# facebookresearch/localrf

Measured on AMD Instinct MI355X. Metric: rays/sec (4096-ray batch, 512 samples, 300^3 grid), higher is better.
Workload: dtype f32 (colour network: split-bf16 3-term products on v_mfma_f32_32x32x16_bf16, fp32 accumulate, <= 3e-5 vs the exact-fp32 engine; gathers and compositing fp32); 1 GPU; configs[1]: single 300^3 TensorVMSplit, 4096 rays x 512 samples per GPU, full density+appearance+MLP render, eval forward; rays_per_gpu=4096, samples_per_ray=512, grid=300, parallelism=ray-shard x1, mlp_engine=bf16x3

## Files before the change

include/lrf_debug.h:

```cpp
#ifndef LRF_DEBUG_H_
#define LRF_DEBUG_H_

#include <stdint.h>

#ifdef __cplusplus
extern "C" {
#endif

void    lrf_debug_set_dump(float* buf);
void    lrf_debug_set_lds_lines(int on);
void    lrf_debug_set_pipe_chunk(int rays);
void    lrf_debug_set_scene_fuse(int on);
void    lrf_debug_set_bwd_overlap(int on);
void    lrf_debug_set_train_fwd_engine(int bits);
void    lrf_debug_set_scatter_wgs(int n);
int64_t lrf_debug_saved_row_offset(int buffer, uint64_t row, int col);

#ifdef __cplusplus
}
#endif
#endif
```

localrf_amd/_native.py:

```python
import ctypes as C
import os

_HERE = os.path.dirname(os.path.abspath(__file__))
LIB_PATH = os.environ.get("LRF_LIB", os.path.join(_HERE, "csrc", "liblrf_hip.so"))

LRF_FLAG_WHITE_BG = 1
LRF_FLAG_RELU_DENS = 2
LRF_FLAG_MLP_VALU = 4
LRF_FLAG_MLP_F32 = 8
LRF_FLAG_ROWS_SAVED = 16
LRF_FLAG_SORT_RAYS = 32
LRF_FLAG_PE_OFF = 64
LRF_FLAG_PLANE_EVENTS = 128
LRF_FLAG_DETERMINISTIC = 256
LRF_FLAG_ALL = 511

_f = C.c_void_p


class LrfParams(C.Structure):
    _fields_ = [("density_plane", _f * 3), ("density_line", _f * 3),
                ("app_plane", _f * 3), ("app_line", _f * 3),
                ("basis", _f), ("w1", _f), ("b1", _f), ("w2", _f), ("b2", _f), ("w3", _f), ("b3", _f),
                ("grid", C.c_int32 * 3), ("fea_pe", C.c_int32), ("view_pe", C.c_int32), ("feature_c", C.c_int32)]
# ... 35 lines not shown

class LrfFlowLoss(C.Structure):
    _fields_ = [("cam2world", _f), ("frame", C.c_void_p), ("fwd_off", C.c_void_p), ("dirs", _f), ("depth", _f), ("ij", C.c_void_p),
                ("fwd_flow", _f), ("fwd_mask", _f), ("bwd_flow", _f), ("bwd_mask", _f), ("focal", _f), ("center", _f),
                ("F", C.c_int32), ("V", C.c_int32), ("n", C.c_int32), ("quantile", C.c_float)]


LRF_LOSS_MAX_PER_VIEW = 4096
LRF_LOSS_TERMS_MAX = 8


class LrfBatchGather(C.Structure):
    _fields_ = [("images", _f), ("fwd_flow", _f), ("bwd_flow", _f), ("invdepths", _f), ("view_ids", C.c_void_p), ("pix", C.c_void_p),
                ("V", C.c_int32), ("n", C.c_int32), ("HW", C.c_int32), ("n_images", C.c_int32)]


class LrfLossTerms(C.Structure):
    _fields_ = [("x", _f * LRF_LOSS_TERMS_MAX), ("n", C.c_int32 * LRF_LOSS_TERMS_MAX), ("a", C.c_float * LRF_LOSS_TERMS_MAX),
                ("b", C.c_float * LRF_LOSS_TERMS_MAX), ("count", C.c_int32), ("s", _f)]


class LrfImageMetrics(C.Structure):
    _fields_ = [("img0", _f), ("img1", _f), ("B", C.c_int32), ("H", C.c_int32), ("W", C.c_int32), ("filter_size", C.c_int32),
                ("max_val", C.c_double), ("filter_sigma", C.c_double), ("k1", C.c_double), ("k2", C.c_double)]


LRF_FRAMES_ERR_NOT_RESIDENT = 1


class LrfFrameWindow(C.Structure):
    _fields_ = [("rgb", _f), ("loss_weight", _f), ("invdepth", _f), ("fwd_flow", _f), ("fwd_mask", _f), ("bwd_flow", _f),
                ("bwd_mask", _f), ("slot_of", C.c_void_p), ("status", C.c_void_p),
                ("capacity", C.c_int32), ("n_px", C.c_int32), ("num_images", C.c_int32)]


LRF_SELECT_QUANTILE = 0
LRF_SELECT_MEDIAN = 1
LRF_SELECT_MAX_ROWS = 256
LRF_EVAL_MAX_VIEWS = 64


class LrfFlowComparison(C.Structure):
    _fields_ = [("cam2world", _f), ("depth", _f), ("dirs", _f), ("ij", C.c_void_p), ("fwd_flow", _f), ("fwd_mask", _f),
                ("bwd_flow", _f), ("bwd_mask", _f), ("focal", _f), ("center", _f),
                ("F", C.c_int32), ("V", C.c_int32), ("H", C.c_int32), ("W", C.c_int32), ("idx", C.c_int32 * LRF_EVAL_MAX_VIEWS)]


SYMBOLS = {
    "lrf_abi_version": (C.c_int, []),
    "lrf_last_error": (C.c_char_p, []),
    "lrf_error_slot": (C.c_void_p, []),
    "lrf_debug_set_dump": (None, [C.c_void_p]),
    "lrf_debug_set_lds_lines": (None, [C.c_int]),
    "lrf_debug_set_pipe_chunk": (None, [C.c_int]),
    "lrf_debug_set_scene_fuse": (None, [C.c_int]),
    "lrf_debug_saved_row_offset": (C.c_int64, [C.c_int, C.c_uint64, C.c_int]),
    "lrf_debug_set_bwd_overlap": (None, [C.c_int]),
    "lrf_debug_set_train_fwd_engine": (None, [C.c_int]),
    "lrf_debug_set_scatter_wgs": (None, [C.c_int]),
    "lrf_workspace_layout_bwd": (None, [C.c_int32, C.c_int32, C.POINTER(C.c_int32), C.POINTER(C.c_uint64)]),
    "lrf_cache_bytes": (C.c_size_t, [C.POINTER(C.c_int32)]),
    "lrf_pack_field": (C.c_int, [C.POINTER(LrfParams), C.c_void_p, C.c_void_p]),
    "lrf_workspace_bytes": (C.c_size_t, [C.c_int32, C.c_int32]),
    "lrf_render_fwd": (C.c_int, [C.POINTER(LrfField), _f, _f, C.c_int32, C.c_int32, C.c_uint32, C.c_float,
                                 _f, _f, _f, _f, C.c_void_p, C.c_void_p]),
    "lrf_render_fwd_profile": (C.c_int, [C.POINTER(LrfField), _f, _f, C.c_int32, C.c_int32, C.c_uint32,
                                         C.c_float, _f, _f, C.c_void_p, C.c_void_p,
                                         C.POINTER(C.c_float), C.POINTER(C.c_int32)]),
    "lrf_render_fwd_train": (C.c_int, [C.POINTER(LrfField), _f, _f, C.c_int32, C.c_int32, C.c_uint32, _f, _f,
                                       C.c_void_p, C.c_void_p]),
    "lrf_workspace_bytes_bwd": (C.c_size_t, [C.c_int32, C.c_int32, C.POINTER(C.c_int32)]),
    "lrf_workspace_bytes_bwd_cfg": (C.c_size_t, [C.c_int32, C.c_int32, C.POINTER(C.c_int32), C.c_int32, C.c_int32, C.c_int32, C.c_uint32]),
    "lrf_render_bwd": (C.c_int, [C.POINTER(LrfField), C.POINTER(LrfParams), _f, _f, C.c_int32, C.c_int32,
                                 C.c_uint32, _f, _f, C.POINTER(LrfGrads), _f, C.c_void_p, C.c_void_p]),
    "lrf_render_bwd_wait": (C.c_int, [C.c_int32, C.c_void_p]),
    "lrf_density_feature": (C.c_int, [C.POINTER(LrfField), _f, C.c_int32, _f, C.c_void_p]),
    "lrf_app_feature": (C.c_int, [C.POINTER(LrfField), _f, C.c_int32, _f, C.c_void_p]),
    "lrf_sample_ray_aabb": (C.c_int, [_f, C.POINTER(C.c_float), C.c_float, C.c_float, C.c_float, _f,
                                      C.c_int32, C.c_int32, _f, _f, C.c_void_p, C.c_void_p]),
    "lrf_sample_ray_contracted": (C.c_int, [_f, _f, _f, C.c_int32, C.c_int32, _f, C.c_void_p]),
    "lrf_z_schedule": (C.c_int, [C.c_int32, _f, _f, _f, C.c_void_p]),
    "lrf_adam_step": (C.c_int, [C.POINTER(LrfAdamTensor), C.c_int32, C.c_float, C.c_float, C.c_float, C.c_void_p]),
    "lrf_adam_step_pack": (C.c_int, [C.POINTER(LrfAdamTensor), C.c_int32, _f, C.c_float, C.c_float, C.c_float, C.POINTER(LrfParams), C.c_void_p, C.c_void_p]),
    "lrf_photo_loss_fwd": (C.c_int, [_f, _f, _f, _f, C.c_int32, _f, _f, C.c_void_p]),
    "lrf_photo_loss_bwd": (C.c_int, [_f, _f, _f, _f, _f, C.c_int32, _f, C.c_void_p]),
    "lrf_batch_gather": (C.c_int, [C.POINTER(LrfBatchGather), _f, _f, _f, _f, _f, _f, C.c_void_p]),
    "lrf_loss_combine_fwd": (C.c_int, [C.POINTER(LrfLossTerms), _f, _f, C.c_void_p]),
    "lrf_loss_combine_bwd": (C.c_int, [_f, _f, C.c_int32, _f, C.c_void_p]),
    "lrf_rows_gather": (C.c_int, [_f, C.c_void_p, C.c_int32, C.c_int32, C.c_int32, _f, C.c_void_p]),
    "lrf_rows_gather_bwd": (C.c_int, [_f, C.c_void_p, C.c_int32, C.c_int32, C.c_int32, _f, C.c_void_p]),
    "lrf_adam_step_dev": (C.c_int, [C.POINTER(LrfAdamTensor), C.c_int32, _f, C.c_float, C.c_float, C.c_float, C.c_void_p]),
    "lrf_density_l1_workspace": (C.c_size_t, [C.POINTER(C.c_int32), C.POINTER(C.c_int32)]),
    "lrf_density_l1_fwd": (C.c_int, [C.POINTER(_f), C.POINTER(_f), C.POINTER(C.c_int32), C.POINTER(C.c_int32),
                                     C.c_float, C.c_int32, C.c_void_p, _f, C.c_void_p]),
    "lrf_density_l1_bwd": (C.c_int, [C.POINTER(_f), C.POINTER(_f), C.POINTER(C.c_int32), C.POINTER(C.c_int32),
                                     C.c_void_p, _f, C.POINTER(_f), C.POINTER(_f), C.c_void_p]),
    "lrf_density_l1_bwd_acc": (C.c_int, [C.POINTER(_f), C.POINTER(_f), C.POINTER(C.c_int32), C.POINTER(C.c_int32),
                                     C.c_void_p, _f, C.POINTER(_f), C.POINTER(_f), C.c_void_p]),
    "lrf_pose_assemble": (C.c_int, [C.POINTER(_f), C.POINTER(_f), C.c_int32, C.c_int32, _f, C.c_void_p]),
    "lrf_pose_assemble_bwd": (C.c_int, [C.POINTER(_f), C.c_int32, C.c_int32, _f, _f, _f, C.c_void_p]),
    "lrf_dense_alpha": (C.c_int, [C.POINTER(LrfField), _f, _f, _f, C.c_int32, C.c_int32, C.c_int32, C.c_float,
                                  C.c_uint32, _f, C.c_void_p]),
    "lrf_alpha_pool_threshold": (C.c_int, [_f, C.c_int32, C.c_int32, C.c_int32, C.c_float, _f, C.c_void_p]),
    "lrf_tv_workspace": (C.c_size_t, [C.POINTER(LrfTvSeg), C.c_int32]),
    "lrf_tv_loss_fwd": (C.c_int, [C.POINTER(LrfTvSeg), C.c_int32, C.c_float, C.c_void_p, _f, C.c_void_p]),
    "lrf_tv_loss_bwd": (C.c_int, [C.POINTER(LrfTvSeg), C.c_int32, C.c_float, _f, C.c_void_p]),
# ... 72 lines not shown
```

localrf_amd/csrc/lrf_common.h:

```cpp
#pragma once
#include "lrf_tu.h"
#include <hip/hip_runtime.h>
#include <stdint.h>
#include "../../include/lrf.h"

namespace lrf {

constexpr int MAT0[3] = {0, 0, 1};
constexpr int MAT1[3] = {1, 2, 2};
constexpr int VEC[3]  = {2, 1, 0};

constexpr int LRF_CAS = 32;
__host__ __device__ constexpr int app_pc(int c) { return 8 * (c / 6) + c % 6; }

constexpr int IMG_BAS  = 0;
constexpr int IMG_W1   = IMG_BAS + 2 * 3 * 64 * 8;
constexpr int IMG_W2   = IMG_W1 + 8 * 2 * 64 * 4;
constexpr int IMG_W3H  = IMG_W2 + 8 * 8 * 64 * 4;
constexpr int IMG_B1   = IMG_W3H + 4 * 32 * 4;
constexpr int IMG_B2   = IMG_B1 + 128;
constexpr int IMG_W3V  = IMG_B2 + 128;
constexpr int IMG_FLOATS = IMG_W3V + 16;

constexpr int IMGB_BAS = 0;
// ... 57 lines not shown
  return (row >> 4) * (size_t)(16 * ld) + (size_t)((col >> 4) * 256 + ((((col >> 2) & 3) * 16 + (int)(row & 15)) << 2) + (col & 3));
}
__device__ __forceinline__ float* frag_lane_base(float* buf, size_t tile, int ld, int s, int g) {
  return buf + tile * (size_t)(16 * ld) + ((g * 16 + s) << 2);
}
__device__ __forceinline__ const float* grd_dx_row(const float* grd, size_t row) {
  return grd + (row >> 4) * (size_t)(16 * GRD_LD) + GRD_DX * 16 + (row & 15) * (GRD_LD - GRD_DX);
}
__device__ __forceinline__ const float* grd_dx8(const float* grd, size_t row, int p, int grp) {
  return grd + (row >> 4) * (size_t)(16 * GRD_LD) + GRD_DX * 16 + (((p * 3 + grp) * 16 + (int)(row & 15)) << 3);
}

struct DField {
  const float* dplane[3]; const float* dline[3];
  const float* aplane[3]; const float* aline[3];
  const float* mlp;
  const uint4* mlpb;
  const float* aplane2[3]; const float* aline2[3];
  const uint4* mlpw;
  const uint4* mlpwt;
  int pw[3], ph[3], ll[3];
  const float* alpha_vol; int ax, ay, az;
  float m_lo[3], m_inv[3];
  float lo[3], inv[3];
  float hi[3];
  float density_shift, distance_scale, weight_thres;
  float term_T;
  const float* basis; const float* w1; const float* b1; const float* w2; const float* b2;
  const float* w3; const float* b3;
  int fea_pe, view_pe, fc;
  float* dump;
  float* rdir;
  const int* perm;
};

__device__ __forceinline__ void contract3(float& x, float& y, float& z) {
  float m = fmaxf(fmaxf(fabsf(x), fabsf(y)), fabsf(z));
  m = fmaxf(m, 1e-6f);
  if (m > 1.0f) {
    const float s = (2.0f * m - 1.0f) / (m * m);
    x *= s; y *= s; z *= s;
  }
}

__device__ __forceinline__ void tap1d(float u, int size, int& i0, int& i1, float& t) {
  float ix = ((u + 1.0f) * 0.5f) * (float)(size - 1);
  ix = fminf(fmaxf(ix, 0.0f), (float)(size - 1));
  const float f0 = floorf(ix);
  t = ix - f0;
  i0 = (int)f0;
  i1 = min(i0 + 1, size - 1);
}

struct AxisTaps { int i0[3], i1[3]; float t[3]; };
__device__ __forceinline__ AxisTaps axis_taps(const int pw0, const int ph0, const int ll0, const float u[3]) {
  AxisTaps a;
  tap1d(u[0], pw0, a.i0[0], a.i1[0], a.t[0]);
  tap1d(u[1], ph0, a.i0[1], a.i1[1], a.t[1]);
  tap1d(u[2], ll0, a.i0[2], a.i1[2], a.t[2]);
  return a;
}

__device__ __forceinline__ float feature2density(float f, float shift, bool relu) {
  if (relu) return fmaxf(f, 0.0f);
  const float y = f + shift;
  return y > 20.0f ? y : log1pf(expf(y));
}

__device__ __forceinline__ float alpha_mask_sample(const DField& f, float x, float y, float z) {
  const float ux = (x - f.m_lo[0]) * f.m_inv[0] - 1.0f;
  const float uy = (y - f.m_lo[1]) * f.m_inv[1] - 1.0f;
  const float uz = (z - f.m_lo[2]) * f.m_inv[2] - 1.0f;
  const float ix = ((ux + 1.0f) * 0.5f) * (float)(f.ax - 1);
  const float iy = ((uy + 1.0f) * 0.5f) * (float)(f.ay - 1);
  const float iz = ((uz + 1.0f) * 0.5f) * (float)(f.az - 1);
  const float fx = floorf(ix), fy = floorf(iy), fz = floorf(iz);
  const float tx = ix - fx, ty = iy - fy, tz = iz - fz;
  const int x0 = (int)fx, y0 = (int)fy, z0 = (int)fz;
  float out = 0.0f;
#pragma unroll
  for (int dz = 0; dz < 2; ++dz)
#pragma unroll
    for (int dy = 0; dy < 2; ++dy)
#pragma unroll
      for (int dx = 0; dx < 2; ++dx) {
        const int xi = x0 + dx, yi = y0 + dy, zi = z0 + dz;
        if (xi >= 0 && xi < f.ax && yi >= 0 && yi < f.ay && zi >= 0 && zi < f.az) {
          const float w = (dx ? tx : 1.0f - tx) * (dy ? ty : 1.0f - ty) * (dz ? tz : 1.0f - tz);
          out += f.alpha_vol[((size_t)zi * f.ay + yi) * f.ax + xi] * w;
        }
      }
  return out;
}

__device__ __forceinline__ void sample_point(const DField& f, const float o[3], const float dh[3],
                                             float zk, float x[3], float u[3]) {
  x[0] = o[0] + dh[0] * zk; x[1] = o[1] + dh[1] * zk; x[2] = o[2] + dh[2] * zk;
  contract3(x[0], x[1], x[2]);
#pragma unroll
  for (int a = 0; a < 3; ++a) u[a] = (x[a] - f.lo[a]) * f.inv[a] - 1.0f;
}

__device__ __forceinline__ float4 ld4(const float* p) { return *reinterpret_cast<const float4*>(p); }
__device__ __forceinline__ float2 ld2(const float* p) { return *reinterpret_cast<const float2*>(p); }

__device__ __forceinline__ float density_feature(const DField& f, const float u[3]) {
  float feat = 0.0f;
#pragma unroll
  for (int p = 0; p < 3; ++p) {
    int x0, x1, y0, y1, l0, l1; float tx, ty, tl;
    tap1d(u[MAT0[p]], f.pw[p], x0, x1, tx);
    tap1d(u[MAT1[p]], f.ph[p], y0, y1, ty);
    tap1d(u[VEC[p]],  f.ll[p], l0, l1, tl);
    const float* pl = f.dplane[p];
    const float* q00 = pl + ((size_t)y0 * f.pw[p] + x0) * LRF_CD;
    const float* q10 = pl + ((size_t)y0 * f.pw[p] + x1) * LRF_CD;
    const float* q01 = pl + ((size_t)y1 * f.pw[p] + x0) * LRF_CD;
    const float* q11 = pl + ((size_t)y1 * f.pw[p] + x1) * LRF_CD;
    const float* r0 = f.dline[p] + (size_t)l0 * LRF_CD;
    const float* r1 = f.dline[p] + (size_t)l1 * LRF_CD;
    const float w00 = (1.0f - tx) * (1.0f - ty), w10 = tx * (1.0f - ty);
    const float w01 = (1.0f - tx) * ty,          w11 = tx * ty;
    const float wl0 = 1.0f - tl, wl1 = tl;
    float sp = 0.0f;
#pragma unroll
    for (int h = 0; h < LRF_CD / 4; ++h) {
      const float4 a = ld4(q00 + 4 * h), b = ld4(q10 + 4 * h), c = ld4(q01 + 4 * h), d = ld4(q11 + 4 * h);
      const float4 e = ld4(r0 + 4 * h), g = ld4(r1 + 4 * h);
      sp += (a.x * w00 + b.x * w10 + c.x * w01 + d.x * w11) * (e.x * wl0 + g.x * wl1);
      sp += (a.y * w00 + b.y * w10 + c.y * w01 + d.y * w11) * (e.y * wl0 + g.y * wl1);
      sp += (a.z * w00 + b.z * w10 + c.z * w01 + d.z * w11) * (e.z * wl0 + g.z * wl1);
      sp += (a.w * w00 + b.w * w10 + c.w * w01 + d.w * w11) * (e.w * wl0 + g.w * wl1);
    }
    feat += sp;
  }
  return feat;
}

__device__ __forceinline__ float4 ld4b(const float* base, unsigned byte_off) {
  return *reinterpret_cast<const float4*>(reinterpret_cast<const char*>(base) + byte_off);
}

__device__ __forceinline__ float density_feature32(const DField& f, const float u[3]) {
  float feat = 0.0f;
#pragma unroll
  for (int p = 0; p < 3; ++p) {
    int x0, x1, y0, y1, l0, l1; float tx, ty, tl;
    tap1d(u[MAT0[p]], f.pw[p], x0, x1, tx);
    tap1d(u[MAT1[p]], f.ph[p], y0, y1, ty);
    tap1d(u[VEC[p]],  f.ll[p], l0, l1, tl);
    const unsigned row0 = (unsigned)y0 * (unsigned)f.pw[p], row1 = (unsigned)y1 * (unsigned)f.pw[p];
    const unsigned o00 = (row0 + x0) * (LRF_CD * 4u), o10 = (row0 + x1) * (LRF_CD * 4u);
    const unsigned o01 = (row1 + x0) * (LRF_CD * 4u), o11 = (row1 + x1) * (LRF_CD * 4u);
    const unsigned q0 = (unsigned)l0 * (LRF_CD * 4u), q1 = (unsigned)l1 * (LRF_CD * 4u);
    const float w00 = (1.0f - tx) * (1.0f - ty), w10 = tx * (1.0f - ty);
    const float w01 = (1.0f - tx) * ty,          w11 = tx * ty;
    const float wl0 = 1.0f - tl, wl1 = tl;
    float sp = 0.0f;
#pragma unroll
    for (int h = 0; h < LRF_CD / 4; ++h) {
      const float4 a = ld4b(f.dplane[p], o00 + 16 * h), b = ld4b(f.dplane[p], o10 + 16 * h);
      const float4 c = ld4b(f.dplane[p], o01 + 16 * h), d = ld4b(f.dplane[p], o11 + 16 * h);
      const float4 e = ld4b(f.dline[p], q0 + 16 * h), g = ld4b(f.dline[p], q1 + 16 * h);
      sp += (a.x * w00 + b.x * w10 + c.x * w01 + d.x * w11) * (e.x * wl0 + g.x * wl1);
      sp += (a.y * w00 + b.y * w10 + c.y * w01 + d.y * w11) * (e.y * wl0 + g.y * wl1);
      sp += (a.z * w00 + b.z * w10 + c.z * w01 + d.z * w11) * (e.z * wl0 + g.z * wl1);
      sp += (a.w * w00 + b.w * w10 + c.w * w01 + d.w * w11) * (e.w * wl0 + g.w * wl1);
    }
    feat += sp;
  }
  return feat;
}

typedef float f32x2 __attribute__((ext_vector_type(2)));
template <bool LDSL>
__device__ __forceinline__ float density_feature_m(const DField& f, const float u[3], const float* const s_line[3]) {
  f32x2 acc = {0.0f, 0.0f};
  const AxisTaps at = axis_taps(f.pw[0], f.ph[0], f.ll[0], u);
#pragma unroll
  for (int p = 0; p < 3; ++p) {
    const int x0 = at.i0[MAT0[p]], x1 = at.i1[MAT0[p]], y0 = at.i0[MAT1[p]], y1 = at.i1[MAT1[p]];
    const int l0 = at.i0[VEC[p]], l1 = at.i1[VEC[p]];
    const float tx = at.t[MAT0[p]], ty = at.t[MAT1[p]], tl = at.t[VEC[p]];
    const unsigned row0 = (unsigned)y0 * (unsigned)f.pw[p], row1 = (unsigned)y1 * (unsigned)f.pw[p];
    const unsigned o00 = (row0 + x0) * (LRF_CD * 4u), o10 = (row0 + x1) * (LRF_CD * 4u);
    const unsigned o01 = (row1 + x0) * (LRF_CD * 4u), o11 = (row1 + x1) * (LRF_CD * 4u);
    const f32x2 w00 = {(1.0f - tx) * (1.0f - ty), (1.0f - tx) * (1.0f - ty)}, w10 = {tx * (1.0f - ty), tx * (1.0f - ty)};
    const f32x2 w01 = {(1.0f - tx) * ty, (1.0f - tx) * ty}, w11 = {tx * ty, tx * ty};
    const f32x2 wl0 = {1.0f - tl, 1.0f - tl}, wl1 = {tl, tl};
#pragma unroll
    for (int h = 0; h < LRF_CD / 4; ++h) {
      const float4 a = ld4b(f.dplane[p], o00 + 16 * h), b = ld4b(f.dplane[p], o10 + 16 * h);
      const float4 c = ld4b(f.dplane[p], o01 + 16 * h), d = ld4b(f.dplane[p], o11 + 16 * h);
      float4 e, g;
      if (LDSL) {
        e = *reinterpret_cast<const float4*>(s_line[p] + l0 * LRF_CD + 4 * h);
        g = *reinterpret_cast<const float4*>(s_line[p] + l1 * LRF_CD + 4 * h);
      } else {
        e = ld4b(f.dline[p], (unsigned)l0 * (LRF_CD * 4u) + 16 * h);
        g = ld4b(f.dline[p], (unsigned)l1 * (LRF_CD * 4u) + 16 * h);
      }
      const f32x2 a0 = {a.x, a.y}, a1 = {a.z, a.w}, b0 = {b.x, b.y}, b1 = {b.z, b.w};
      const f32x2 c0 = {c.x, c.y}, c1 = {c.z, c.w}, d0 = {d.x, d.y}, d1 = {d.z, d.w};
      const f32x2 e0 = {e.x, e.y}, e1 = {e.z, e.w}, g0 = {g.x, g.y}, g1 = {g.z, g.w};
      acc += (a0 * w00 + b0 * w10 + c0 * w01 + d0 * w11) * (e0 * wl0 + g0 * wl1);
      acc += (a1 * w00 + b1 * w10 + c1 * w01 + d1 * w11) * (e1 * wl0 + g1 * wl1);
    }
  }
  return acc.x + acc.y;
}

__device__ __forceinline__ void wave_scan_prod(float v, int lane, float& excl, float& total) {
  float p = v;
#pragma unroll
  for (int d = 1; d < 64; d <<= 1) {
    const float t = __shfl_up(p, d, 64);
    if (lane >= d) p *= t;
  }
  excl = __shfl_up(p, 1, 64);
  if (lane == 0) excl = 1.0f;
  total = __shfl(p, 63, 64);
}

__device__ __forceinline__ float wave_sum(float v) {
#pragma unroll
  for (int d = 32; d >= 1; d >>= 1) v += __shfl_xor(v, d, 64);
  return v;
}

}
```

localrf_amd/csrc/lrf_render.hip:

```cpp
#include <hip/hip_runtime.h>
#include <stdint.h>
#include <stdio.h>
#include <string.h>
#include <stdlib.h>
#include <mutex>
#include "lrf_common.h"

namespace lrf {

constexpr int ITEM = 16;

thread_local char g_err[512] = "";
static int set_err(const char* msg, hipError_t e = hipSuccess) {
  char* slot = lrf_error_slot();
  if (e != hipSuccess) snprintf(slot, 512, "%s: %s", msg, hipGetErrorString(e));
  else snprintf(slot, 512, "%s", msg);
  return 1;
}
#define LRF_HIP(call) do { hipError_t e_ = (call); if (e_ != hipSuccess) return set_err(#call, e_); } while (0)

struct PackSeg { const float* src; float* dst; int C, H, W, CS, app; };
struct PackTab { PackSeg s[18]; };
struct PackMlp { float* mlp; uint32_t* mlpb; uint32_t* mlpw; uint32_t* mlpwt; int mode; };
__device__ void pack_mlp_elem(const LrfParams& p, float* __restrict__ img, int idx);
// ... 139 lines not shown
    out[h] = part ? bf16_bits(v - bf16_val(hi)) : hi;
  }
  img[idx] = (uint32_t)out[0] | ((uint32_t)out[1] << 16);
}

__device__ void pack_mlp_w32_elem(const LrfParams& p, uint32_t* __restrict__ img, int idx) {
  if (idx >= W32_ALL_U4 * 4) return;
  if (idx >= W32_U4 * 4) {
    const int e = idx - W32_U4 * 4;
    float v = 0.0f;
    if (e < W32_T_B2) v = p.b1[e - W32_T_B1];
    else if (e < W32_T_W3) v = p.b2[e - W32_T_B2];
    else if (e < W32_T_B3) {
      const int c = (e - W32_T_W3) / W32_T_W3_LD, u = (e - W32_T_W3) % W32_T_W3_LD;
      if (u < LRF_FEATC + 3) v = p.w3[c * (LRF_FEATC + 3) + u];
    } else if (e < W32_T_B3 + 3) v = p.b3[e - W32_T_B3];
    img[idx] = __float_as_uint(v);
    return;
  }
  const int u4 = idx >> 2, wj = idx & 3;
  const int lane = u4 & 63, part = (u4 >> 6) & 1, frag = u4 >> 7;
  const int n = lane & 31, h = lane >> 5;
  unsigned short out[2];
#pragma unroll
  for (int hh = 0; hh < 2; ++hh) {
    const int j = 2 * wj + hh;
    float v = 0.0f;
    if (frag < W32_W1) {
      const int c = w32_chan(h, 8 * frag + j);
      if (c >= 0 && n < LRF_APP_DIM) v = p.basis[n * 72 + c];
    } else if (frag < W32_W2) {
      const int e = frag - W32_W1, m = e >> 1, q = e & 1;
      const int u = w32_unit(0, q, h, j);
      if (u < LRF_APP_DIM) v = p.w1[(32 * m + n) * LRF_APP_DIM + u];
    } else {
      const int e = frag - W32_W2, m = e >> 3, m0 = (e >> 1) & 3, q = e & 1;
      v = p.w2[(32 * m + n) * LRF_FEATC + w32_unit(m0, q, h, j)];
    }
    const unsigned short hi = bf16_bits(v);
    out[hh] = part ? bf16_bits(v - bf16_val(hi)) : hi;
  }
  img[idx] = (uint32_t)out[0] | ((uint32_t)out[1] << 16);
}

constexpr int LRF_MULTI_MAX = 4;
struct MultiF { DField f[LRF_MULTI_MAX]; int nf, Rf, Rs, lo; };
__device__ __forceinline__ int multi_io(const MultiF& m, int k, int vray) { return k * m.Rs + m.lo + (vray - k * m.Rf); }
template <bool MULTI> struct FieldArg { typedef DField type; };
template <> struct FieldArg<true> { typedef MultiF type; };
__device__ __forceinline__ const DField& field_of(const DField& f, int) { return f; }
__device__ __forceinline__ const DField& field_of(const MultiF& m, int k) { return m.f[k]; }

template <bool LDSL, bool MULTI = false>
__global__ __launch_bounds__(1024) void k_march(
    typename FieldArg<MULTI>::type fin, const float* __restrict__ rays, const float* __restrict__ z, int R, int S,
    uint32_t flags, float floater,
    float* __restrict__ depth, float* __restrict__ acc_ws, float* __restrict__ w_all,
    int* __restrict__ ncomp, uint16_t* __restrict__ cidx, float* __restrict__ cw,
    float* __restrict__ feat_out ) {
  extern __shared__ float s_alpha_all[];
  const int wave = threadIdx.x >> 6, lane = threadIdx.x & 63;
  const int nb = gridDim.x;
  const int lb = (nb % 8 == 0) ? (int)(blockIdx.x % 8) * (nb / 8) + (int)(blockIdx.x / 8) : (int)blockIdx.x;
  const int nw = blockDim.x >> 6;
  const int ray = lb * nw + wave;
  int fk_ = 0;
  if constexpr (MULTI) fk_ = min((lb * nw) / fin.Rf, fin.nf - 1);
  const DField& f = field_of(fin, fk_);
  int io_ray = ray;
  if constexpr (MULTI) io_ray = multi_io(fin, fk_, ray);
  const float* s_line[3] = {nullptr, nullptr, nullptr};
  if (LDSL) {
    float* base = s_alpha_all + (size_t)nw * S;
#pragma unroll
    for (int p = 0; p < 3; ++p) {
      const int n = f.ll[p] * LRF_CD / 4;
      float4* dst = reinterpret_cast<float4*>(base);
      const float4* src = reinterpret_cast<const float4*>(f.dline[p]);
      for (int i = threadIdx.x; i < n; i += blockDim.x) dst[i] = src[i];
      s_line[p] = base;
      base += f.ll[p] * LRF_CD;
    }
    __syncthreads();
  }
  if (ray >= R) return;
  float* s_alpha = s_alpha_all + (size_t)wave * S;
  const int oray = f.perm ? f.perm[ray] : io_ray;

  const float* rp = rays + (size_t)io_ray * 6;
  const float o[3] = {rp[0], rp[1], rp[2]};
  const float dn = sqrtf(rp[3] * rp[3] + rp[4] * rp[4] + rp[5] * rp[5]);
  const float dh[3] = {rp[3] / dn, rp[4] / dn, rp[5] / dn};
  const bool relu = flags & LRF_FLAG_RELU_DENS;
  const int nchunk = (S + 63) >> 6;

  {
    float carry = 1.0f;
    bool live = true;
    for (int c = 0; c < nchunk; ++c) {
      const int k = (c << 6) + lane;
      float alpha = 0.0f, fk = -INFINITY;
      if (live && k < S - 1) {
        const float zk = z[k];
        float x[3], u[3];
        sample_point(f, o, dh, zk, x, u);
        bool valid = true;
        if (f.alpha_vol) valid = alpha_mask_sample(f, x[0], x[1], x[2]) > 0.0f;
        if (valid) {
          fk = density_feature_m<LDSL>(f, u, s_line);
          const float sigma = feature2density(fk, f.density_shift, relu);
          const float dist = z[k + 1] - zk;
          alpha = 1.0f - expf(-sigma * dist * f.distance_scale);
        }
      }
      if (k < S) {
        s_alpha[k] = alpha;
        if (feat_out) feat_out[(size_t)ray * S + k] = fk;
      }
      if (live && f.term_T > 0.0f) {
        float v = (k < S - 1) ? (1.0f - alpha + 1e-10f) : 1.0f;
#pragma unroll
        for (int d = 32; d >= 1; d >>= 1) v *= __shfl_xor(v, d, 64);
        carry *= v;
        if (__builtin_amdgcn_readfirstlane(__float_as_int(carry)) < __float_as_int(f.term_T)) live = false;
      }
    }
  }

  float acc = 0.0f, dsum = 0.0f, kbar = 0.0f;
  int nsh = 0;
  const int npass = floater > 0.0f ? 2 : 1;
  for (int pass = 0; pass < npass; ++pass) {
    const bool emit = (pass == npass - 1);
    float carry = 1.0f, a_acc = 0.0f, a_d = 0.0f, a_k = 0.0f;
    for (int c = 0; c < nchunk; ++c) {
      const int k = (c << 6) + lane;
      float alpha = 0.0f;
      if (k < S) {
        alpha = s_alpha[k];
        if (pass == 1 && (float)k < kbar * floater) alpha = 0.0f;
        if (k == S - 1) alpha = 1.0f;
      }
      const float v = (k < S) ? (1.0f - alpha + 1e-10f) : 1.0f;
      float excl, total;
      wave_scan_prod(v, lane, excl, total);
      const float T = carry * excl;
      carry *= total;
      const float w = alpha * T;
      if (pass == 0) {
        a_acc += w;
        a_d += (k < S) ? w * z[k] : 0.0f;
        a_k += w * (float)k;
      }
      if (emit) {
        if (w_all && k < S) w_all[(size_t)oray * S + k] = w;
        const bool sh = (k < S) && (w > f.weight_thres);
        const unsigned long long m = __ballot(sh);
        if (sh) {
          const int pos = nsh + __popcll(m & ((1ull << lane) - 1ull));
          cidx[(size_t)ray * S + pos] = (uint16_t)k;
          cw[(size_t)ray * S + pos] = w;
        }
        nsh += __popcll(m);
      }
    }
    if (pass == 0) {
      acc = wave_sum(a_acc);
      dsum = wave_sum(a_d);
      kbar = wave_sum(a_k);
    }
  }
  if (lane == 0) {
    depth[oray] = dsum / dn;
    acc_ws[ray] = acc;
    ncomp[ray] = nsh;
    if (f.rdir) *reinterpret_cast<float4*>(f.rdir + (size_t)ray * 4) = make_float4(dh[0], dh[1], dh[2], dn);
  }
}

__global__ __launch_bounds__(1024) void k_scan_tiles(const int* __restrict__ ncomp, int R, int* __restrict__ toff) {
  __shared__ int s_wave[16];
  __shared__ int s_carry;
  const int tid = threadIdx.x, lane = tid & 63, wave = tid >> 6;
  if (tid == 0) s_carry = 0;
  __syncthreads();
  for (int base = 0; base < R; base += 1024) {
    const int r = base + tid;
    const int v = r < R ? (ncomp[r] + ITEM - 1) / ITEM : 0;
    int incl = v;
#pragma unroll
    for (int d = 1; d < 64; d <<= 1) {
      const int t = __shfl_up(incl, d, 64);
      if (lane >= d) incl += t;
    }
    if (lane == 63) s_wave[wave] = incl;
    __syncthreads();
    int woff = 0;
    for (int q = 0; q < wave; ++q) woff += s_wave[q];
    const int carry = s_carry;
    if (r < R) toff[r] = carry + woff + incl - v;
    __syncthreads();
    if (tid == 1023) s_carry = carry + woff + incl;
    __syncthreads();
  }
  if (tid == 0) toff[R] = s_carry;
}

typedef float f32x4 __attribute__((ext_vector_type(4)));

__device__ __forceinline__ f32x4 mfma4(float a, float b, f32x4 c) {
  return __builtin_amdgcn_mfma_f32_16x16x4f32(a, b, c, 0, 0, 0);
}

template <int p>
__device__ __forceinline__ void gather_app6_plane(const DField& f, const float u[3], int g, float X[8]) {
  int x0, x1, y0, y1, l0, l1; float tx, ty, tl;
  tap1d(u[MAT0[p]], f.pw[p], x0, x1, tx);
  tap1d(u[MAT1[p]], f.ph[p], y0, y1, ty);
  tap1d(u[VEC[p]],  f.ll[p], l0, l1, tl);
  const float* pl = f.aplane[p] + 8 * g;
  const float* q00 = pl + ((size_t)y0 * f.pw[p] + x0) * LRF_CAS;
  const float* q10 = pl + ((size_t)y0 * f.pw[p] + x1) * LRF_CAS;
  const float* q01 = pl + ((size_t)y1 * f.pw[p] + x0) * LRF_CAS;
  const float* q11 = pl + ((size_t)y1 * f.pw[p] + x1) * LRF_CAS;
  const float* r0 = f.aline[p] + (size_t)l0 * LRF_CAS + 8 * g;
  const float* r1 = f.aline[p] + (size_t)l1 * LRF_CAS + 8 * g;
  const float w00 = (1.0f - tx) * (1.0f - ty), w10 = tx * (1.0f - ty);
  const float w01 = (1.0f - tx) * ty,          w11 = tx * ty;
  const float wl0 = 1.0f - tl, wl1 = tl;
// ... 357 lines not shown
  }
  d.mlp = base + L.mlp;
  d.mlpb = reinterpret_cast<const uint4*>(base + L.mlpb);
  for (int p = 0; p < 3; ++p) { d.aplane2[p] = base + L.aplane2[p]; d.aline2[p] = base + L.aline2[p]; }
  d.mlpw = reinterpret_cast<const uint4*>(base + L.mlpw);
  d.mlpwt = reinterpret_cast<const uint4*>(base + L.mlpwt);
  d.alpha_vol = f->alpha_vol;
  d.ax = f->alpha_dim[0]; d.ay = f->alpha_dim[1]; d.az = f->alpha_dim[2];
  for (int a = 0; a < 3; ++a) {
    d.lo[a] = f->aabb[a];
    d.hi[a] = f->aabb[3 + a];
    d.inv[a] = 2.0f / (f->aabb[3 + a] - f->aabb[a]);
    d.m_lo[a] = f->alpha_aabb[a];
    d.m_inv[a] = 1.0f / (f->alpha_aabb[3 + a] - f->alpha_aabb[a]) * 2.0f;
  }
  d.density_shift = f->density_shift; d.distance_scale = f->distance_scale; d.weight_thres = f->weight_thres;
  d.term_T = f->term_T > 0.0f ? f->term_T : 0.0f;
  d.dump = nullptr;
  d.rdir = nullptr;
  d.perm = nullptr;
  d.basis = f->basis; d.w1 = f->w1; d.b1 = f->b1; d.w2 = f->w2; d.b2 = f->b2; d.w3 = f->w3; d.b3 = f->b3;
  d.fea_pe = f->fea_pe; d.view_pe = f->view_pe; d.fc = f->feature_c ? f->feature_c : LRF_FEATC;
  return d;
}

struct Workspace {
  int* toff; int* ncomp; float* acc; uint16_t* cidx; float* cw; float* part;
  float* rdir;
  int* perm; float* rays_s;
  int pmax; size_t bytes;
};
static size_t up256(size_t x) { return (x + 255) & ~size_t(255); }
static Workspace carve(void* ws, int R, int S) {
  Workspace w;
  char* p = reinterpret_cast<char*>(ws);
  size_t off = 0;
  w.pmax = 2 * ((S + ITEM3 - 1) / ITEM3);
  w.toff  = reinterpret_cast<int*>(p + off);       off += up256((size_t)(R + 1) * 4);
  w.ncomp = reinterpret_cast<int*>(p + off);       off += up256((size_t)R * 4);
  w.acc   = reinterpret_cast<float*>(p + off);     off += up256((size_t)R * 4);
  w.cidx  = reinterpret_cast<uint16_t*>(p + off);  off += up256((size_t)R * S * 2);
  w.cw    = reinterpret_cast<float*>(p + off);     off += up256((size_t)R * S * 4);
  w.part  = reinterpret_cast<float*>(p + off);     off += up256((size_t)R * w.pmax * 12);
  w.rdir  = reinterpret_cast<float*>(p + off);     off += up256((size_t)R * 16);
  w.perm  = reinterpret_cast<int*>(p + off);       off += up256((size_t)R * 4);
  w.rays_s = reinterpret_cast<float*>(p + off);    off += up256((size_t)R * 24);
  w.bytes = off;
  return w;
}

static float* g_dump = nullptr;
static int g_no_lds_lines = 0;
static int g_pipe_chunk = 16384;
static int g_no_scene_fuse = 0;

static int device_cus() {
  static int cache[64] = {};
  int dev = 0;
  if (hipGetDevice(&dev) != hipSuccess) return 256;
  int& cus = cache[dev & 63];
  if (!cus) {
    hipDeviceProp_t prop;
    if (hipGetDeviceProperties(&prop, dev) == hipSuccess) cus = prop.multiProcessorCount;
    if (cus <= 0) cus = 256;
  }
  return cus;
}

static int g_bwd_overlap = 1;
struct SideStream { hipStream_t s; hipEvent_t fork, join, app[2], bucket[5]; bool ok, bucket_set; std::mutex mu; };
static SideStream* side_stream() {
  static SideStream tab[64];
  static std::mutex init_mu;
  int dev = 0;
  if (hipGetDevice(&dev) != hipSuccess) return nullptr;
  SideStream& x = tab[dev & 63];
  std::lock_guard<std::mutex> lk(init_mu);
  if (!x.ok) {
    if (hipStreamCreateWithFlags(&x.s, hipStreamNonBlocking) != hipSuccess) return nullptr;
    if (hipEventCreateWithFlags(&x.fork, hipEventDisableTiming) != hipSuccess ||
        hipEventCreateWithFlags(&x.join, hipEventDisableTiming) != hipSuccess ||
        hipEventCreateWithFlags(&x.app[0], hipEventDisableTiming) != hipSuccess ||
        hipEventCreateWithFlags(&x.app[1], hipEventDisableTiming) != hipSuccess) return nullptr;
    for (int q = 0; q < 5; ++q)
      if (hipEventCreateWithFlags(&x.bucket[q], hipEventDisableTiming) != hipSuccess) return nullptr;
    x.bucket_set = false;
    x.ok = true;
  }
  return &x;
}
static hipError_t lds_opt_in();

constexpr int LRF_SORT_MAX_R = 32768;
static bool sorts_rays(int R, uint32_t flags) { return (flags & LRF_FLAG_SORT_RAYS) && R >= 2 && R <= LRF_SORT_MAX_R; }
static const float* sort_rays_if_asked(DField& d, const float* rays, int R, uint32_t flags, const Workspace& w, hipStream_t st) {
  d.perm = nullptr;
  if (!sorts_rays(R, flags)) return rays;
  int N = 2;
  while (N < R) N <<= 1;
  hipLaunchKernelGGL(k_sort_rays, dim3(1), dim3(1024), (size_t)N * 4, st, rays, R, N, w.rays_s, w.perm);
  d.perm = w.perm;
  return w.rays_s;
}

static int march_lds_rays(const int32_t ll[3], int S) {
  if (g_no_lds_lines) return 0;
  const size_t lds_l = (size_t)(ll[0] + ll[1] + ll[2]) * LRF_CD * sizeof(float);
  for (int cand = 4; cand <= 16; cand *= 2)
    if (((size_t)cand * S * sizeof(float) + lds_l) * (16 / cand) <= 156 * 1024) return cand;
  return 0;
}
static void launch_march(const DField& d, const float* rays, const float* z, int R, int S, uint32_t flags, float floater,
                         float* depth, float* acc, float* w_all, int* ncomp, uint16_t* cidx, float* cw, float* feat,
                         hipStream_t st, const MultiF* mf = nullptr) {
  const size_t lds_l = (size_t)(d.ll[0] + d.ll[1] + d.ll[2]) * LRF_CD * sizeof(float);
  const int nw = march_lds_rays(d.ll, S);
  if (nw) {
    const size_t lds = (size_t)nw * S * sizeof(float) + lds_l;
    if (mf) {
      hipLaunchKernelGGL((k_march<true, true>), dim3((R + nw - 1) / nw), dim3(64 * nw), lds, st,
                         *mf, rays, z, R, S, flags, floater, depth, acc, w_all, ncomp, cidx, cw, feat);
      return;
    }
    hipLaunchKernelGGL(k_march<true>, dim3((R + nw - 1) / nw), dim3(64 * nw), lds, st,
                       d, rays, z, R, S, flags, floater, depth, acc, w_all, ncomp, cidx, cw, feat);
  } else {
    hipLaunchKernelGGL(k_march<false>, dim3((R + 3) / 4), dim3(256), (size_t)4 * S * sizeof(float), st,
                       d, rays, z, R, S, flags, floater, depth, acc, w_all, ncomp, cidx, cw, feat);
  }
}

static void launch_shade3(DField d, const float* rays, const float* z, int R, int S, uint32_t flags, const Workspace& w,
                         int* toff32, float* rgb, float* acc_out, const SaveOut3* sv, float* dump, hipStream_t st) {
  const size_t lds_base = (size_t)W32_ALL_U4 * sizeof(uint4) + (size_t)S * sizeof(float);
  const size_t lds_toff = (size_t)(R + 1) * sizeof(int) + (size_t)R * sizeof(unsigned short) + 16;
  const bool in_lds = lds_base + lds_toff + 64 <= 160 * 1024 - 256;
  const dim3 grid(device_cus()), block(512);
  if (sv) {
    if (in_lds) {
      hipLaunchKernelGGL((k_shade3<8, true, false, true>), grid, block, lds_base + lds_toff, st,
                         d, rays, z, S, toff32, R, w.ncomp, w.cidx, w.cw, w.part, w.pmax, flags, w.acc, rgb, acc_out, *sv);
    } else {
      hipLaunchKernelGGL(k_scan_tiles_n<ITEM3>, dim3(1), dim3(1024), 0, st, w.ncomp, R, toff32);
      hipLaunchKernelGGL((k_shade3<8, false, false, true>), grid, block, lds_base, st,
                         d, rays, z, S, toff32, R, w.ncomp, w.cidx, w.cw, w.part, w.pmax, flags, w.acc, rgb, acc_out, *sv);
    }
  } else if (in_lds && dump) {
    d.dump = dump;
    hipLaunchKernelGGL((k_shade3<8, true, true>), grid, block, lds_base + lds_toff, st,
                       d, rays, z, S, toff32, R, w.ncomp, w.cidx, w.cw, w.part, w.pmax, flags, w.acc, rgb, acc_out, SaveOut3{});
  } else if (in_lds) {
    hipLaunchKernelGGL((k_shade3<8, true, false>), grid, block, lds_base + lds_toff, st,
                       d, rays, z, S, toff32, R, w.ncomp, w.cidx, w.cw, w.part, w.pmax, flags, w.acc, rgb, acc_out, SaveOut3{});
  } else {
    hipLaunchKernelGGL(k_scan_tiles_n<ITEM3>, dim3(1), dim3(1024), 0, st, w.ncomp, R, toff32);
    hipLaunchKernelGGL((k_shade3<8, false, false>), grid, block, lds_base, st,
                       d, rays, z, S, toff32, R, w.ncomp, w.cidx, w.cw, w.part, w.pmax, flags, w.acc, rgb, acc_out, SaveOut3{});
  }
}

static void launch_shade3_multi(const MultiF& mf, const float* rays, const float* z, int Rv, int S, uint32_t flags,
                                const Workspace& w, float* rgb, hipStream_t st) {
  const size_t lds_base = (size_t)W32_ALL_U4 * sizeof(uint4) + (size_t)S * sizeof(float);
  hipLaunchKernelGGL(k_scan_tiles_n<ITEM3>, dim3(1), dim3(1024), 0, st, w.ncomp, Rv, w.toff);
  hipLaunchKernelGGL((k_shade3m<8, false>), dim3(device_cus()), dim3(512), lds_base, st,
                     mf, rays, z, S, w.toff, Rv, w.ncomp, w.cidx, w.cw, w.part, w.pmax, flags, w.acc, rgb, (float*)nullptr, SaveOut3{});
}

}

#include "lrf_generic.inl"
namespace lrf {
static const char* gen_check(const LrfField* f) {
  const int fc = f->feature_c ? f->feature_c : LRF_FEATC;
  if (f->fea_pe < 0 || f->fea_pe > GEN_MAX_PE || f->view_pe < 0 || f->view_pe > GEN_MAX_PE || fc < 1 || fc > GEN_MAX_FC)
    return "localrf: unsupported colour-network configuration (need 0 <= fea_pe, view_pe <= 6 and 1 <= featureC <= 256)";
  if (!gen_is_default(f->fea_pe, f->view_pe, fc) && (!f->basis || !f->w1 || !f->b1 || !f->w2 || !f->b2 || !f->w3 || !f->b3))
    return "localrf: a non-default colour-network configuration needs the natural-layout weights in LrfField (basis, w1 .. b3)";
  return nullptr;
}
static hipError_t launch_shade_gen(const DField& d, const GenCfg& gc, const float* rays, const float* z, int R, int S, const Workspace& w,
// ... 26 lines not shown
    {reinterpret_cast<const void*>(&k_gen_dgrad<32>), L160 - 1024},
    {reinterpret_cast<const void*>(&k_gen_dgrad<16>), L160 - 1024},
    {reinterpret_cast<const void*>(&k_scatter_plane<LRF_CA, true, LRF_APP_NT, false>), L160},
    {reinterpret_cast<const void*>(&k_scatter_plane<LRF_CA, true, LRF_APP_NT, true>), L160},
    {reinterpret_cast<const void*>(&k_scatter_plane<LRF_CD, false, 512, true>), L160},
    {reinterpret_cast<const void*>(&k_scatter_line<LRF_CA, true, 1024>), L160},
    {reinterpret_cast<const void*>(&k_scatter_line<LRF_CD, false, 1024>), L160},
    {reinterpret_cast<const void*>(&k_bwd_ray), 14 * LRF_MAX_S_TRAIN * 4 + BIN_MAX * 4},
    {reinterpret_cast<const void*>(&k_train_dgrad3<8>), L160 - 256},
    {reinterpret_cast<const void*>(&k_train_app3<8, false>), 128 * 1024},
    {reinterpret_cast<const void*>(&k_train_app3<8, true>), 128 * 1024},
    {reinterpret_cast<const void*>(&k_scatter_fix<LRF_CD, false, FIX_NT>), L160},
    {reinterpret_cast<const void*>(&k_scatter_fix<LRF_CA, true, FIX_NT>), L160},
    {reinterpret_cast<const void*>(&k_scatter_fix<LRF_CA, true, FIX_NT, 4>), L160},
    {reinterpret_cast<const void*>(&k_scatter_det<LRF_CD, false, FIX_NT>), L160},
    {reinterpret_cast<const void*>(&k_scatter_det<LRF_CA, true, FIX_NT>), L160},
    {reinterpret_cast<const void*>(&k_scatter_det<LRF_CA, true, FIX_NT, 4>), L160},
    {reinterpret_cast<const void*>(&k_wgrad_w2w3<128>), (int)w23_lds(128)},
    {reinterpret_cast<const void*>(&k_wgrad_w2w3<64>), (int)w23_lds(64)},
  };
  static std::once_flag once[64];
  static hipError_t err[64];
  int dev = 0;
  const hipError_t e0 = hipGetDevice(&dev);
  if (e0 != hipSuccess) return e0;
  std::call_once(once[dev & 63], [dev] {
    hipError_t e = hipSuccess;
    for (const auto& t : tab)
      if (e == hipSuccess) e = hipFuncSetAttribute(t.k, hipFuncAttributeMaxDynamicSharedMemorySize, t.bytes);
    err[dev & 63] = e;
  });
  return err[dev & 63];
}
}
#include "lrf_scene.inl"
#include "lrf_adam.inl"
#include "lrf_losses.inl"
#include "lrf_metrics.inl"
#include "lrf_frames.inl"
#include "lrf_select.inl"
#include "lrf_evalgeo.inl"
#include "lrf_encode.inl"
#include "lrf_reg.inl"
#include "lrf_mask.inl"

using namespace lrf;

extern "C" {

int lrf_abi_version(void) { return LRF_ABI_VERSION; }
void lrf_debug_set_dump(float* buf) { g_dump = buf; }
void lrf_debug_set_bwd_overlap(int on) { g_bwd_overlap = (on & 1) ? 1 : 0; if (on > 1) g_wgrad_split = (on >> 1) - 1; }
void lrf_debug_set_lds_lines(int on) { g_no_lds_lines = on ? 0 : 1; }
void lrf_debug_set_pipe_chunk(int rays) { g_pipe_chunk = rays > 0 ? rays : 0; }
#ifdef LRF_SCATTER_PROF
int lrf_debug_scatter_prof(unsigned long long* host_out ) {
  return (int)hipMemcpyFromSymbol(host_out, HIP_SYMBOL(lrf::g_scat_prof), sizeof(unsigned long long) * 2 * 2048 * 12);
}
#endif
void lrf_debug_set_scene_fuse(int on) { g_no_scene_fuse = on ? 0 : 1; }
int64_t lrf_debug_saved_row_offset(int buffer, uint64_t row, int col) {
  using namespace lrf;
  if (buffer == 0) return (col < 0 || col >= ACT_LD) ? -1 : (int64_t)frag_off((size_t)row, col, ACT_LD);
  if (buffer == 1) {
    if (col < 0 || col >= GRD_LD) return -1;
    if (col >= GRD_DX) return (int64_t)((row >> 4) * (uint64_t)(16 * GRD_LD) + GRD_DX * 16 + (row & 15) * (GRD_LD - GRD_DX) + (col - GRD_DX));
    return (int64_t)frag_off((size_t)row, col, GRD_LD);
  }
  return -1;
}
const char* lrf_last_error(void) { return lrf_error_slot(); }
char* lrf_error_slot(void) { return g_err; }

size_t lrf_cache_bytes(const int32_t grid[3]) { return make_layout(grid).total * sizeof(float); }

int lrf_pack_field(const LrfParams* p, void* cache, void* stream) {
  if (!p || !cache) return set_err("lrf_pack_field: null argument");
  hipStream_t st = reinterpret_cast<hipStream_t>(stream);
  const Layout L = make_layout(p->grid);
  float* base = reinterpret_cast<float*>(cache);
  PackTab tab;
  int wmax = 1, hmax = 1;
  for (int q = 0; q < 3; ++q) {
    tab.s[4 * q + 0] = PackSeg{p->density_plane[q], base + L.dplane[q], LRF_CD, L.ph[q], L.pw[q], LRF_CD, 0};
    tab.s[4 * q + 1] = PackSeg{p->app_plane[q], base + L.aplane[q], LRF_CA, L.ph[q], L.pw[q], LRF_CAS, 1};
    tab.s[4 * q + 2] = PackSeg{p->density_line[q], base + L.dline[q], LRF_CD, 1, L.ll[q], LRF_CD, 0};
    tab.s[4 * q + 3] = PackSeg{p->app_line[q], base + L.aline[q], LRF_CA, 1, L.ll[q], LRF_CAS, 1};
    tab.s[12 + 2 * q + 0] = PackSeg{p->app_plane[q], base + L.aplane2[q], LRF_CA, L.ph[q], L.pw[q], LRF_CA, 0};
    tab.s[12 + 2 * q + 1] = PackSeg{p->app_line[q], base + L.aline2[q], LRF_CA, 1, L.ll[q], LRF_CA, 0};
    wmax = max(wmax, max(L.pw[q], L.ll[q]));
    hmax = max(hmax, L.ph[q]);
  }
  static_assert(IMG_FLOATS <= 26880 && IMGB_ALL * 4 <= 26880 && W32_ALL_U4 * 4 <= 26880 && W32T_ALL_U4 * 4 <= 26880, "slice 18 of k_pack_planes covers every network image");
  PackMlp pm;
  pm.mlp = base + L.mlp; pm.mlpb = reinterpret_cast<uint32_t*>(base + L.mlpb); pm.mlpw = reinterpret_cast<uint32_t*>(base + L.mlpw);
  pm.mlpwt = reinterpret_cast<uint32_t*>(base + L.mlpwt);
  pm.mode = gen_is_default(p->fea_pe, p->view_pe, p->feature_c ? p->feature_c : LRF_FEATC) ? 0 : 1;
  hipLaunchKernelGGL(k_pack_planes, dim3((wmax + 127) / 128, hmax, 19), dim3(128), 0, st, tab, *p, pm, 0);
  LRF_HIP(hipGetLastError());
  return 0;
}

static int pipe_chunks(int R) { return (g_pipe_chunk > 0 && R >= 2 * g_pipe_chunk) ? (R + g_pipe_chunk - 1) / g_pipe_chunk : 1; }
size_t lrf_workspace_bytes(int32_t R, int32_t S) {
  const size_t whole = carve(nullptr, R, S).bytes;
  const int nc = pipe_chunks(R);
// ... 230 lines not shown
```

Measured before the change: 25.15 million rays/s.

## Split march chunks across waves per ray and pin march occupancy

Adds an opt-in mode in which several waves march one ray, each taking interleaved 64-sample chunks. Early termination is coordinated through per-chunk transmittance products kept in LDS, and a final pass zeroes the samples past the termination point. The default path also changes: k_march gets an amdgpu_waves_per_eu(8,8) occupancy pin, and ray origin, norm and grid-extent values are marked wave-uniform with readfirstlane. A sched_barrier is added in the density gather loop, and the rdir write moves ahead of the march. The occupancy pin caps registers and may cause spills, and the scheduling barrier can reduce instruction overlap.

```diff
diff --git a/include/lrf_debug.h b/include/lrf_debug.h
--- a/include/lrf_debug.h
+++ b/include/lrf_debug.h
@@ -9,6 +9,7 @@
 
 void    lrf_debug_set_dump(float* buf);
 void    lrf_debug_set_lds_lines(int on);
+void    lrf_debug_set_march_waves(int w);
 void    lrf_debug_set_pipe_chunk(int rays);
 void    lrf_debug_set_scene_fuse(int on);
 void    lrf_debug_set_bwd_overlap(int on);
diff --git a/localrf_amd/_native.py b/localrf_amd/_native.py
--- a/localrf_amd/_native.py
+++ b/localrf_amd/_native.py
@@ -111,6 +111,7 @@
     "lrf_error_slot": (C.c_void_p, []),
     "lrf_debug_set_dump": (None, [C.c_void_p]),
     "lrf_debug_set_lds_lines": (None, [C.c_int]),
+    "lrf_debug_set_march_waves": (None, [C.c_int]),
     "lrf_debug_set_pipe_chunk": (None, [C.c_int]),
     "lrf_debug_set_scene_fuse": (None, [C.c_int]),
     "lrf_debug_saved_row_offset": (C.c_int64, [C.c_int, C.c_uint64, C.c_int]),
diff --git a/localrf_amd/csrc/lrf_common.h b/localrf_amd/csrc/lrf_common.h
--- a/localrf_amd/csrc/lrf_common.h
+++ b/localrf_amd/csrc/lrf_common.h
@@ -133,6 +133,8 @@
   i1 = min(i0 + 1, size - 1);
 }
 
+__device__ __forceinline__ float uniform_f(float v) { return __int_as_float(__builtin_amdgcn_readfirstlane(__float_as_int(v))); }
+
 struct AxisTaps { int i0[3], i1[3]; float t[3]; };
 __device__ __forceinline__ AxisTaps axis_taps(const int pw0, const int ph0, const int ll0, const float u[3]) {
   AxisTaps a;
@@ -152,9 +154,9 @@
   const float ux = (x - f.m_lo[0]) * f.m_inv[0] - 1.0f;
   const float uy = (y - f.m_lo[1]) * f.m_inv[1] - 1.0f;
   const float uz = (z - f.m_lo[2]) * f.m_inv[2] - 1.0f;
-  const float ix = ((ux + 1.0f) * 0.5f) * (float)(f.ax - 1);
-  const float iy = ((uy + 1.0f) * 0.5f) * (float)(f.ay - 1);
-  const float iz = ((uz + 1.0f) * 0.5f) * (float)(f.az - 1);
+  const float ix = ((ux + 1.0f) * 0.5f) * uniform_f((float)(f.ax - 1));
+  const float iy = ((uy + 1.0f) * 0.5f) * uniform_f((float)(f.ay - 1));
+  const float iz = ((uz + 1.0f) * 0.5f) * uniform_f((float)(f.az - 1));
   const float fx = floorf(ix), fy = floorf(iy), fz = floorf(iz);
   const float tx = ix - fx, ty = iy - fy, tz = iz - fz;
   const int x0 = (int)fx, y0 = (int)fy, z0 = (int)fz;
@@ -257,7 +259,19 @@
 template <bool LDSL>
 __device__ __forceinline__ float density_feature_m(const DField& f, const float u[3], const float* const s_line[3]) {
   f32x2 acc = {0.0f, 0.0f};
-  const AxisTaps at = axis_taps(f.pw[0], f.ph[0], f.ll[0], u);
+  AxisTaps at;
+  {
+    const int n[3] = {f.pw[0], f.ph[0], f.ll[0]};
+#pragma unroll
+    for (int a = 0; a < 3; ++a) {
+      const float top = uniform_f((float)(n[a] - 1));
+      const float ix = fminf(fmaxf(((u[a] + 1.0f) * 0.5f) * top, 0.0f), top);
+      const float f0 = floorf(ix);
+      at.t[a] = ix - f0;
+      at.i0[a] = (int)f0;
+      at.i1[a] = min(at.i0[a] + 1, n[a] - 1);
+    }
+  }
 #pragma unroll
   for (int p = 0; p < 3; ++p) {
     const int x0 = at.i0[MAT0[p]], x1 = at.i1[MAT0[p]], y0 = at.i0[MAT1[p]], y1 = at.i1[MAT1[p]];
@@ -286,6 +300,7 @@
       const f32x2 e0 = {e.x, e.y}, e1 = {e.z, e.w}, g0 = {g.x, g.y}, g1 = {g.z, g.w};
       acc += (a0 * w00 + b0 * w10 + c0 * w01 + d0 * w11) * (e0 * wl0 + g0 * wl1);
       acc += (a1 * w00 + b1 * w10 + c1 * w01 + d1 * w11) * (e1 * wl0 + g1 * wl1);
+      __builtin_amdgcn_sched_barrier(0);
     }
   }
   return acc.x + acc.y;
diff --git a/localrf_amd/csrc/lrf_render.hip b/localrf_amd/csrc/lrf_render.hip
--- a/localrf_amd/csrc/lrf_render.hip
+++ b/localrf_amd/csrc/lrf_render.hip
@@ -215,26 +215,30 @@
 __device__ __forceinline__ const DField& field_of(const MultiF& m, int k) { return m.f[k]; }
 
 template <bool LDSL, bool MULTI = false>
-__global__ __launch_bounds__(1024) void k_march(
+__global__ __launch_bounds__(1024) __attribute__((amdgpu_waves_per_eu(8, 8))) void k_march(
     typename FieldArg<MULTI>::type fin, const float* __restrict__ rays, const float* __restrict__ z, int R, int S,
     uint32_t flags, float floater,
     float* __restrict__ depth, float* __restrict__ acc_ws, float* __restrict__ w_all,
     int* __restrict__ ncomp, uint16_t* __restrict__ cidx, float* __restrict__ cw,
-    float* __restrict__ feat_out ) {
+    float* __restrict__ feat_out , int wsh) {
   extern __shared__ float s_alpha_all[];
-  const int wave = threadIdx.x >> 6, lane = threadIdx.x & 63;
+  const int wave = __builtin_amdgcn_readfirstlane(threadIdx.x >> 6), lane = threadIdx.x & 63;
   const int nb = gridDim.x;
   const int lb = (nb % 8 == 0) ? (int)(blockIdx.x % 8) * (nb / 8) + (int)(blockIdx.x / 8) : (int)blockIdx.x;
-  const int nw = blockDim.x >> 6;
-  const int ray = lb * nw + wave;
+  const int wpr = 1 << wsh;
+  const int nw = blockDim.x >> (6 + wsh);
+  const int rw = wave >> wsh, sub = wave & (wpr - 1);
+  const int ray = lb * nw + rw;
   int fk_ = 0;
   if constexpr (MULTI) fk_ = min((lb * nw) / fin.Rf, fin.nf - 1);
   const DField& f = field_of(fin, fk_);
   int io_ray = ray;
   if constexpr (MULTI) io_ray = multi_io(fin, fk_, ray);
+  const int nchunk = (S + 63) >> 6;
+  const bool term = f.term_T > 0.0f;
   const float* s_line[3] = {nullptr, nullptr, nullptr};
+  float* base = s_alpha_all + (size_t)nw * S;
   if (LDSL) {
-    float* base = s_alpha_all + (size_t)nw * S;
 #pragma unroll
     for (int p = 0; p < 3; ++p) {
       const int n = f.ll[p] * LRF_CD / 4;
@@ -244,23 +248,37 @@
       s_line[p] = base;
       base += f.ll[p] * LRF_CD;
     }
-    __syncthreads();
-  }
-  if (ray >= R) return;
-  float* s_alpha = s_alpha_all + (size_t)wave * S;
-  const int oray = f.perm ? f.perm[ray] : io_ray;
-
-  const float* rp = rays + (size_t)io_ray * 6;
-  const float o[3] = {rp[0], rp[1], rp[2]};
-  const float dn = sqrtf(rp[3] * rp[3] + rp[4] * rp[4] + rp[5] * rp[5]);
+  }
+  volatile float* s_prod = base + (size_t)rw * nchunk;
+  if (wpr > 1 && term)
+    for (int i = threadIdx.x; i < nw * nchunk; i += blockDim.x) base[i] = -1.0f;
+  if (LDSL || wpr > 1) __syncthreads();
+  const bool in_batch = ray < R;
+  if (wpr == 1 && !in_batch) return;
+  float* s_alpha = s_alpha_all + (size_t)rw * S;
+  const int oray = f.perm ? f.perm[in_batch ? ray : 0] : io_ray;
+
+  const float* rp = rays + (size_t)(in_batch ? io_ray : 0) * 6;
+  const float o[3] = {uniform_f(rp[0]), uniform_f(rp[1]), uniform_f(rp[2])};
+  const float dn = uniform_f(sqrtf(rp[3] * rp[3] + rp[4] * rp[4] + rp[5] * rp[5]));
   const float dh[3] = {rp[3] / dn, rp[4] / dn, rp[5] / dn};
   const bool relu = flags & LRF_FLAG_RELU_DENS;
-  const int nchunk = (S + 63) >> 6;
-
-  {
+  if (lane == 0 && sub == 0 && in_batch && f.rdir) *reinterpret_cast<float4*>(f.rdir + (size_t)ray * 4) = make_float4(dh[0], dh[1], dh[2], dn);
+
+  if (in_batch) {
     float carry = 1.0f;
     bool live = true;
-    for (int c = 0; c < nchunk; ++c) {
+    int cpos = 0;
+    for (int c = sub; c < nchunk; c += wpr) {
+      if (wpr > 1 && term) {
+        while (live && cpos < c) {
+          const float pr = __int_as_float(__builtin_amdgcn_readfirstlane(__float_as_int(s_prod[cpos])));
+          if (pr < 0.0f) break;
+          carry *= pr;
+          ++cpos;
+          if (__builtin_amdgcn_readfirstlane(__float_as_int(carry)) < __float_as_int(f.term_T)) live = false;
+        }
+      }
       const int k = (c << 6) + lane;
       float alpha = 0.0f, fk = -INFINITY;
       if (live && k < S - 1) {
@@ -280,12 +298,33 @@
         s_alpha[k] = alpha;
         if (feat_out) feat_out[(size_t)ray * S + k] = fk;
       }
-      if (live && f.term_T > 0.0f) {
+      if (live && term) {
         float v = (k < S - 1) ? (1.0f - alpha + 1e-10f) : 1.0f;
 #pragma unroll
         for (int d = 32; d >= 1; d >>= 1) v *= __shfl_xor(v, d, 64);
-        carry *= v;
-        if (__builtin_amdgcn_readfirstlane(__float_as_int(carry)) < __float_as_int(f.term_T)) live = false;
+        if (wpr > 1) {
+          if (lane == 0) s_prod[c] = v;
+        } else {
+          carry *= v;
+          if (__builtin_amdgcn_readfirstlane(__float_as_int(carry)) < __float_as_int(f.term_T)) live = false;
+        }
+      }
+    }
+  }
+  if (wpr > 1) {
+    if (feat_out && term) __builtin_amdgcn_s_waitcnt(0x0F70);
+    __syncthreads();
+    if (sub != 0 || !in_batch) return;
+    if (term) {
+      float carry = 1.0f;
+      int cterm = nchunk;
+      for (int c = 0; c < nchunk; ++c) {
+        carry *= __int_as_float(__builtin_amdgcn_readfirstlane(__float_as_int(s_prod[c])));
+        if (__builtin_amdgcn_readfirstlane(__float_as_int(carry)) < __float_as_int(f.term_T)) { cterm = c + 1; break; }
+      }
+      for (int k = (cterm << 6) + lane; k < S; k += 64) {
+        s_alpha[k] = 0.0f;
+        if (feat_out) feat_out[(size_t)ray * S + k] = -INFINITY;
       }
     }
   }
@@ -337,7 +376,6 @@
     depth[oray] = dsum / dn;
     acc_ws[ray] = acc;
     ncomp[ray] = nsh;
-    if (f.rdir) *reinterpret_cast<float4*>(f.rdir + (size_t)ray * 4) = make_float4(dh[0], dh[1], dh[2], dn);
   }
 }
 
@@ -801,6 +839,7 @@
 static float* g_dump = nullptr;
 static int g_no_lds_lines = 0;
 static int g_pipe_chunk = 16384;
+static int g_march_waves = 0;
 static int g_no_scene_fuse = 0;
 
 static int device_cus() {
@@ -859,23 +898,33 @@
     if (((size_t)cand * S * sizeof(float) + lds_l) * (16 / cand) <= 156 * 1024) return cand;
   return 0;
 }
+static int march_wave_shift(int R, int S, int nr) {
+  const int nchunk = (S + 63) / 64;
+  (void)R;
+  const int want = g_march_waves ? g_march_waves : 1;
+  int wsh = 0;
+  while ((2 << wsh) <= want && nr * (2 << wsh) <= 16 && (2 << wsh) <= nchunk) ++wsh;
+  return wsh;
+}
 static void launch_march(const DField& d, const float* rays, const float* z, int R, int S, uint32_t flags, float floater,
                          float* depth, float* acc, float* w_all, int* ncomp, uint16_t* cidx, float* cw, float* feat,
                          hipStream_t st, const MultiF* mf = nullptr) {
   const size_t lds_l = (size_t)(d.ll[0] + d.ll[1] + d.ll[2]) * LRF_CD * sizeof(float);
   const int nw = march_lds_rays(d.ll, S);
   if (nw) {
-    const size_t lds = (size_t)nw * S * sizeof(float) + lds_l;
+    const int wsh = march_wave_shift(R, S, nw);
+    const size_t lds = (size_t)nw * S * sizeof(float) + lds_l + (wsh ? (size_t)nw * ((S + 63) / 64) * sizeof(float) : 0);
+    const dim3 grid((R + nw - 1) / nw), block((64 * nw) << wsh);
     if (mf) {
-      hipLaunchKernelGGL((k_march<true, true>), dim3((R + nw - 1) / nw), dim3(64 * nw), lds, st,
-                         *mf, rays, z, R, S, flags, floater, depth, acc, w_all, ncomp, cidx, cw, feat);
+      hipLaunchKernelGGL((k_march<true, true>), grid, block, lds, st,
+                         *mf, rays, z, R, S, flags, floater, depth, acc, w_all, ncomp, cidx, cw, feat, wsh);
       return;
     }
-    hipLaunchKernelGGL(k_march<true>, dim3((R + nw - 1) / nw), dim3(64 * nw), lds, st,
-                       d, rays, z, R, S, flags, floater, depth, acc, w_all, ncomp, cidx, cw, feat);
+    hipLaunchKernelGGL(k_march<true>, grid, block, lds, st,
+                       d, rays, z, R, S, flags, floater, depth, acc, w_all, ncomp, cidx, cw, feat, wsh);
   } else {
     hipLaunchKernelGGL(k_march<false>, dim3((R + 3) / 4), dim3(256), (size_t)4 * S * sizeof(float), st,
-                       d, rays, z, R, S, flags, floater, depth, acc, w_all, ncomp, cidx, cw, feat);
+                       d, rays, z, R, S, flags, floater, depth, acc, w_all, ncomp, cidx, cw, feat, 0);
   }
 }
 
@@ -1008,6 +1057,7 @@
 void lrf_debug_set_dump(float* buf) { g_dump = buf; }
 void lrf_debug_set_bwd_overlap(int on) { g_bwd_overlap = (on & 1) ? 1 : 0; if (on > 1) g_wgrad_split = (on >> 1) - 1; }
 void lrf_debug_set_lds_lines(int on) { g_no_lds_lines = on ? 0 : 1; }
+void lrf_debug_set_march_waves(int w) { g_march_waves = (w == 1 || w == 2 || w == 4) ? w : 0; }
 void lrf_debug_set_pipe_chunk(int rays) { g_pipe_chunk = rays > 0 ? rays : 0; }
 #ifdef LRF_SCATTER_PROF
 int lrf_debug_scatter_prof(unsigned long long* host_out ) {
```

Result: no change. 25.03 million rays/s (-0.5%).
